# facebookresearch/omni3d

Measured on AMD Instinct MI355X. Metric: images/sec train DLA34_FPN b=4/GPU, higher is better.
Workload: dtype f32; 1 GPU; cubercnn_DLA34_FPN train step, batch 4/GPU, synthetic Omni3D 512x512 (8 GT/img), fwd+10 losses+bwd+allreduce+divergence guard+SGD, random-init weights; global_batch=4, image=512x512, parallelism=dp1 (flat-bucket RCCL all-reduce)

## Files before the change

include/omni3d_hip.h:

```cpp
#ifndef OMNI3D_HIP_H
#define OMNI3D_HIP_H

#ifdef __cplusplus
extern "C" {
#endif


int omni_iou_box3d(const float* boxes1, int N, const float* boxes2, int M, const int* valid1, float* vol,
                   float* iou, int* overflow, void* stream);

int omni_iou_box3d_pairs(const float* boxes1, const float* boxes2, const int* idx1, const int* idx2,
                         long long npairs, const int* valid1, float* vol, float* iou, int* overflow,
                         void* stream);

int omni_iou_box3d_pairs_algo(const float* boxes1, const float* boxes2, const int* idx1, const int* idx2,
                              long long npairs, const int* valid1, float* vol, float* iou, int* overflow,
                              int lanes_per_pair, void* stream);

int omni_box3d_validity(const float* boxes, int N, float eps_coplanar, float eps_nonzero, int* valid,
                        int* counts, void* stream);


int omni_conv2d_fwd(const float* x, const float* w, const float* bias, float* out, int N, int H, int W, int C,
                    int K, int R, int S, int stride, int pad, int ldx, int ldo, int relu, void* stream);
// ... 29 lines not shown
int omni_gemm_batched_split(const float* A, const float* B, float* out, int batch, int M, int N, int K, int terms, void* stream);
int omni_conv2d_s2_dgrad(const float* dy, const float* w, float* dx, int N, int H, int W, int C, int K, int lddy, int lddx,
                         int accumulate, void* stream);
int omni_conv2d_wgrad_multi_det(const void* const* xs, const int* cs, int nsrc, const float* dy, float* dw, int N, int H, int W, int K,
                                int lddy, int accumulate, int tile, float* ws, long long ws_floats, int* ctr, int n_ctr, long long* plan,
                                void* stream);


int omni_bn_fwd_algo(const float* x, const float* partial, int nblk, const float* gamma, const float* beta, const float* residual,
                     float* y, long long ldy, float* running_mean, float* running_var, float* mean_rstd, float* scale_shift,
                     double* ws, int P, int C, float eps, float momentum, int relu, int fuse_rows, void* stream);
int omni_bn_bwd_algo(const float* x, const float* dy, long long lddy, const float* y, const float* gamma, const float* mean_rstd,
                     const float* partial, int nblk, float* dx, float* dres, const float* res_carry, long long ldc, float* dgamma,
                     float* dbeta, double* ws, float* coef, int P, int C, int relu, int accumulate_param_grads, int fuse_rows,
                     void* stream);

int omni_bn_apply(const float* x, const float* scale_shift, const float* residual, float* y, int P, int C,
                  int relu, void* stream);

int omni_bn_frozen_fwd(const float* x, const float* gamma, const float* beta, const float* running_mean, const float* running_var,
                       float eps, const float* residual, float* y, int P, int C, int relu, void* stream);
int omni_bn_frozen_bwd(const float* x, const float* dy, long long lddy, const float* y, const float* gamma, const float* beta,
                       const float* running_mean, const float* running_var, float eps, float* dx, float* dres, const float* res_carry,
                       long long ldc, float* dgamma, float* dbeta, float* ws, long long ws_floats, int P, int C, int relu,
                       int accumulate_param_grads, void* stream);

int omni_maxpool2_fwd(const float* x, float* y, int N, int H, int W, int C, void* stream);
int omni_maxpool2_bwd(const float* x, const float* dy, float* dx, int N, int H, int W, int C, void* stream);

int omni_grouped_conv2d_fwd(const float* x, const float* w, float* out, int N, int H, int W, int C, int K, int R, int S, int stride,
// ... 272 lines not shown
```

omni3d_amd/csrc/bn_pool.hip:

```cpp
#include <device_rt.h>

namespace {

__device__ __forceinline__ float4 ld4(const float* p) { return *reinterpret_cast<const float4*>(p); }
__device__ __forceinline__ void st4(float* p, float4 v) { *reinterpret_cast<float4*>(p) = v; }
__device__ __forceinline__ float4 f4(float a) { return make_float4(a, a, a, a); }
__device__ __forceinline__ float4 relu4(float4 a) { return make_float4(fmaxf(a.x, 0.f), fmaxf(a.y, 0.f), fmaxf(a.z, 0.f), fmaxf(a.w, 0.f)); }
__device__ __forceinline__ float4 mask4(float4 g, float4 y) {
    return make_float4(y.x > 0.f ? g.x : 0.f, y.y > 0.f ? g.y : 0.f, y.z > 0.f ? g.z : 0.f, y.w > 0.f ? g.w : 0.f);
}

template <int MODE>
__device__ __forceinline__ void bn_reduce_tile(const float* __restrict__ x, const float* __restrict__ dy,
                                               const float* __restrict__ y, const float* __restrict__ mean_rstd,
                                               int P, int C, int relu, double* __restrict__ acc, int cbase, int C4,
                                               float4* __restrict__ s0, float4* __restrict__ s1, long lddy) {
    const int rows = 256 / C4;
    const int t = threadIdx.x;
    const int col = cbase + t % C4, row = t / C4;
    const bool active = row < rows;
    float4 a0 = f4(0.f), a1 = f4(0.f);
    float4 mu = f4(0.f), rs = f4(0.f), sc = f4(0.f), sh = f4(0.f);
    if (MODE == 1 && active) { mu = ld4(mean_rstd + 4 * col); rs = ld4(mean_rstd + C + 4 * col); }
    if (MODE == 1 && active && relu == 2) { sc = ld4(y + 4 * col); sh = ld4(y + C + 4 * col); }
// ... 343 lines not shown
        const float4 x0 = ld4(x + p * C + coff), x1 = two ? ld4(x + p1 * C + coff) : f4(0.f);
        if (relu == 1) {
            g0 = mask4(g0, ld4(y + p * C + coff));
            if (two) g1 = mask4(g1, ld4(y + p1 * C + coff));
        } else if (relu == 2) {
            g0 = mask4(g0, x0 * msc + msh);
            g1 = mask4(g1, x1 * msc + msh);
        }
        if (dres != nullptr) {
            st4(dres + p * C + coff, res_carry != nullptr ? g0 + ld4(res_carry + p * ldc + coff) : g0);
            if (two) st4(dres + p1 * C + coff, res_carry != nullptr ? g1 + ld4(res_carry + p1 * ldc + coff) : g1);
        }
        const float4 h0 = (x0 - mu) * rs, h1 = (x1 - mu) * rs;
        st4(dx + p * C + coff, k0 * (g0 - k1 - h0 * k2));
        if (two) st4(dx + p1 * C + coff, k0 * (g1 - k1 - h1 * k2));
    }
}

__device__ __forceinline__ float frozen_rsqrt(float v) {
#ifdef OMNI_HIPEMU
    return 1.f / sqrtf(v);
#else
    return rsqrtf(v);
#endif
}
__device__ __forceinline__ void frozen_coef(const float* __restrict__ gamma, const float* __restrict__ beta,
                                            const float* __restrict__ running_mean, const float* __restrict__ running_var, float eps,
                                            long c, float4& sc, float4& sh, float4& mu, float4& rs) {
#pragma clang fp contract(off)
    const float4 g = ld4(gamma + c), b = ld4(beta + c), v = ld4(running_var + c);
// ... 412 lines not shown
        int CG, PC, chunk, grid;
        fin_geometry(P, C, CG, PC, chunk, grid);
        hipLaunchKernelGGL(bn_fin_bwd_apply_kernel, dim3(grid), dim3(256), 0, st, x, dy, (long)lddy, y, mean_rstd, gamma, partial, nblk, P, C,
                           dgamma, dbeta, accumulate_param_grads, dx, dres, res_carry, (long)ldc, relu, CG, PC, chunk);
        return omni_launch_status();
    }
    if (coef == nullptr) return OMNI_ERR_ARG;
    hipLaunchKernelGGL(bn_finalize_bwd_kernel, dim3((C + FIN_C - 1) / FIN_C), dim3(256), 0, st, partial, nblk, P, C, gamma, mean_rstd,
                       dgamma, dbeta, coef, accumulate_param_grads);
    const long total4 = (long)P * (C >> 2);
    hipLaunchKernelGGL(bn_bwd_apply_kernel, dim3(ew_grid(total4)), dim3(256), 0, st, x, dy, y, mean_rstd,
                       (const float*)coef, dx, dres, total4, C, relu, res_carry, (long)ldc, (long)lddy);
    return omni_launch_status();
}

int omni_bn_frozen_fwd(const float* x, const float* gamma, const float* beta, const float* running_mean, const float* running_var,
                       float eps, const float* residual, float* y, int P, int C, int relu, void* stream) {
    if (P <= 0 || C <= 0 || (C & 3) || C > 4096 || !gamma || !beta || !running_mean || !running_var) return OMNI_ERR_ARG;
    int CG, PC, chunk, grid;
    fin_geometry(P, C, CG, PC, chunk, grid);
    hipLaunchKernelGGL(bn_frozen_fwd_kernel, dim3(grid), dim3(256), 0, (hipStream_t)stream, x, gamma, beta, running_mean, running_var, eps,
                       residual, y, P, C, relu, CG, PC, chunk);
    return omni_launch_status();
}

int omni_bn_frozen_bwd(const float* x, const float* dy, long long lddy, const float* y, const float* gamma, const float* beta,
                       const float* running_mean, const float* running_var, float eps, float* dx, float* dres, const float* res_carry,
                       long long ldc, float* dgamma, float* dbeta, float* ws, long long ws_floats, int P, int C, int relu,
                       int accumulate_param_grads, void* stream) {
    if (P <= 0 || C <= 0 || (C & 3) || C > 4096 || relu < 0 || relu > 2 || (relu == 1 && y == nullptr)) return OMNI_ERR_ARG;
// ... 163 lines not shown
```

omni3d_amd/csrc/winograd.hip:

```cpp
#include <device_rt.h>

namespace {

__device__ __forceinline__ float4 ld4(const float* p) { return *reinterpret_cast<const float4*>(p); }
__device__ __forceinline__ void st4(float* p, float4 v) { *reinterpret_cast<float4*>(p) = v; }
__device__ __forceinline__ float4 z4() { return make_float4(0.f, 0.f, 0.f, 0.f); }

inline int ew_grid(long total) {
    long g = (total + 255) / 256;
    if (g > 4096) g = 4096;
    return (int)(g < 1 ? 1 : g);
}

__device__ __forceinline__ float4 wino_ld(const float* __restrict__ p, bool ok, bool aff, float4 sc, float4 sh, int relu) {
    if (!ok) return z4();
    float4 v = ld4(p);
    if (aff) {
        v = v * sc + sh;
        if (relu) v = make_float4(fmaxf(v.x, 0.f), fmaxf(v.y, 0.f), fmaxf(v.z, 0.f), fmaxf(v.w, 0.f));
    }
    return v;
}

__global__ void __launch_bounds__(256) wino_in_kernel(const float* __restrict__ x, float* __restrict__ V, int N, int H, int W,
// ... 226 lines not shown
__global__ void __launch_bounds__(256) wino_dw_kernel(const float* __restrict__ dU, float* __restrict__ dg, int K, int C,
                                                      int accumulate) {
#pragma clang fp contract(off)
    const long total = (long)K * C;
    for (long i = (long)blockIdx.x * blockDim.x + threadIdx.x; i < total; i += (long)gridDim.x * blockDim.x) {
        const int c = (int)(i % C), k = (int)(i / C);
        float v[3][3];
        wino_dw_elem(dU, total, i, v);
#pragma unroll
        for (int r = 0; r < 3; ++r) {
            float* o = dg + ((long)k * 9 + r * 3) * C + c;
            if (accumulate) { o[0] += v[r][0]; o[C] += v[r][1]; o[2 * (long)C] += v[r][2]; }
            else { o[0] = v[r][0]; o[C] = v[r][1]; o[2 * (long)C] = v[r][2]; }
        }
    }
}

template <typename V>
__device__ __forceinline__ void bt6(const V (&d)[6], V (&t)[6]) {
    t[0] = d[0] + (d[3] - d[1]) * 1.5f - d[2] * 2.f + d[4];
    t[1] = d[2] * 0.5f + d[3] * 2.5f - d[1] + d[4];
    t[2] = d[1] - d[2] * 2.5f + d[3] * 0.5f + d[4];
    t[3] = (d[3] - d[1]) * 2.f - d[2] + d[4];
    t[4] = (d[1] - d[3]) * 0.5f - d[2] + d[4];
    t[5] = d[1] + (d[4] - d[2]) * 1.5f - d[3] * 2.f + d[5];
}
template <typename V>
__device__ __forceinline__ void at6(const V (&m)[6], V (&y)[4]) {
    y[0] = m[0] + m[1] + m[2] + m[3] + m[4];
    y[1] = m[1] - m[2] + m[3] * 0.5f - m[4] * 2.f;
    y[2] = m[1] + m[2] + m[3] * 0.25f + m[4] * 4.f;
    y[3] = m[1] - m[2] + m[3] * 0.125f - m[4] * 8.f + m[5];
}
template <typename V>
__device__ __forceinline__ void a6(const V (&y)[4], V (&u)[6]) {
    u[0] = y[0];
    u[1] = y[0] + y[1] + y[2] + y[3];
    u[2] = y[0] - y[1] + y[2] - y[3];
    u[3] = y[0] + y[1] * 0.5f + y[2] * 0.25f + y[3] * 0.125f;
    u[4] = y[0] - y[1] * 2.f + y[2] * 4.f - y[3] * 8.f;
    u[5] = y[3];
}

__global__ void __launch_bounds__(256) wino4_in_kernel(const float* __restrict__ x, float* __restrict__ V, int N, int H, int W,
                                                       int C, const float* __restrict__ affine, int relu, long plane_in) {
    const int C4 = C >> 2, TH = H >> 2, TW = W >> 2;
    const bool aff = affine != nullptr;
    const long T = (long)N * TH * TW, total = T * C4, plane = plane_in > 0 ? plane_in : T * C;
    for (long i = (long)blockIdx.x * blockDim.x + threadIdx.x; i < total; i += (long)gridDim.x * blockDim.x) {
        const int c4 = (int)(i % C4);
        const long t = i / C4;
        const int tx = (int)(t % TW);
        const int ty = (int)((t / TW) % TH);
        const int n = (int)(t / ((long)TW * TH));
        const float4 sc = aff ? ld4(affine + 4 * c4) : z4(), sh = aff ? ld4(affine + C + 4 * c4) : z4();
        float4 u[6][6];
// ... 337 lines not shown
        const long t = i / K4;
        const int tx = (int)(t % TW);
        const int ty = (int)((t / TW) % TH);
        const int n = (int)(t / ((long)TW * TH));
        float4 d[4][4];
#pragma unroll
        for (int r = 0; r < 4; ++r) {
            const int ih = 2 * ty - 1 + r;
#pragma unroll
            for (int s = 0; s < 4; ++s) {
                const int iw = 2 * tx - 1 + s;
                const bool ok = (unsigned)ih < (unsigned)H && (unsigned)iw < (unsigned)W;
                d[r][s] = ok ? ld4(dy + (((long)n * H + ih) * W + iw) * K + 4 * k4) : z4();
            }
        }
        const long o = t * K + 4 * k4;
        {
            float4 u[4][4];
#pragma unroll
            for (int s = 0; s < 4; ++s) {
                u[0][s] = d[0][s] - d[2][s];
                u[1][s] = d[1][s] + d[2][s];
                u[2][s] = d[2][s] - d[1][s];
                u[3][s] = d[1][s] - d[3][s];
            }
#pragma unroll
            for (int r = 0; r < 4; ++r) {
                st4(Vd + o + (long)(4 * r + 0) * plane, u[r][0] - u[r][2]);
                st4(Vd + o + (long)(4 * r + 1) * plane, u[r][1] + u[r][2]);
                st4(Vd + o + (long)(4 * r + 2) * plane, u[r][2] - u[r][1]);
                st4(Vd + o + (long)(4 * r + 3) * plane, u[r][1] - u[r][3]);
            }
        }
        {
            const float4 g00 = d[1][1], g01 = d[1][2], g10 = d[2][1], g11 = d[2][2];
            float4 u[4][2];
            u[0][0] = g00;        u[0][1] = g01;
            u[1][0] = g00 + g10;  u[1][1] = g01 + g11;
            u[2][0] = g00 - g10;  u[2][1] = g01 - g11;
            u[3][0] = z4() - g10; u[3][1] = z4() - g11;
#pragma unroll
            for (int r = 0; r < 4; ++r) {
                st4(dM + o + (long)(4 * r + 0) * plane, u[r][0]);
                st4(dM + o + (long)(4 * r + 1) * plane, u[r][0] + u[r][1]);
                st4(dM + o + (long)(4 * r + 2) * plane, u[r][0] - u[r][1]);
                st4(dM + o + (long)(4 * r + 3) * plane, z4() - u[r][1]);
            }
        }
    }
}

__global__ void __launch_bounds__(256) wino4_dy_in_kernel(const float* __restrict__ dy, float* __restrict__ dM, float* __restrict__ Vd,
                                                          int N, int H, int W, int K, long plane_in) {
    const int K4 = K >> 2, TH = H >> 2, TW = W >> 2;
    const long T = (long)N * TH * TW, total = T * K4, plane = plane_in > 0 ? plane_in : T * K;
    for (long i = (long)blockIdx.x * blockDim.x + threadIdx.x; i < total; i += (long)gridDim.x * blockDim.x) {
        const int k4 = (int)(i % K4);
        const long t = i / K4;
        const int tx = (int)(t % TW);
        const int ty = (int)((t / TW) % TH);
        const int n = (int)(t / ((long)TW * TH));
        float4 d[6][6];
#pragma unroll
        for (int r = 0; r < 6; ++r) {
            const int ih = 4 * ty - 1 + r;
#pragma unroll
            for (int s = 0; s < 6; ++s) {
                const int iw = 4 * tx - 1 + s;
                const bool ok = (unsigned)ih < (unsigned)H && (unsigned)iw < (unsigned)W;
                d[r][s] = ok ? ld4(dy + (((long)n * H + ih) * W + iw) * K + 4 * k4) : z4();
            }
        }
        const long o = t * K + 4 * k4;
        {
            float4 u[6][4];
#pragma unroll
            for (int c = 0; c < 4; ++c) {
                float4 col[4], o6[6];
#pragma unroll
                for (int r = 0; r < 4; ++r) col[r] = d[1 + r][1 + c];
                a6(col, o6);
#pragma unroll
                for (int r = 0; r < 6; ++r) u[r][c] = o6[r];
            }
#pragma unroll
            for (int r = 0; r < 6; ++r) {
                float4 row[6];
                a6(u[r], row);
#pragma unroll
                for (int c = 0; c < 6; ++c) st4(dM + o + (long)(6 * r + c) * plane, row[c]);
            }
        }
        {
            float4 u[6][6];
#pragma unroll
            for (int s = 0; s < 6; ++s) {
                float4 col[6], tcol[6];
#pragma unroll
                for (int r = 0; r < 6; ++r) col[r] = d[r][s];
                bt6(col, tcol);
#pragma unroll
                for (int r = 0; r < 6; ++r) u[r][s] = tcol[r];
            }
#pragma unroll
            for (int r = 0; r < 6; ++r) {
                float4 v[6];
                bt6(u[r], v);
#pragma unroll
                for (int s = 0; s < 6; ++s) st4(Vd + o + (long)(6 * r + s) * plane, v[s]);
            }
        }
    }
}

inline bool bad(int N, int H, int W, int C) { return N < 0 || H <= 0 || W <= 0 || C <= 0 || (C & 3); }

}

extern "C" {

int omni_wino_in(const float* x, float* V, int N, int H, int W, int C, int tile, void* stream) {
    if (bad(N, H, W, C) || (tile != 2 && tile != 4) || (H % tile) || (W % tile)) return OMNI_ERR_ARG;
    const long total = (long)N * (H / tile) * (W / tile) * (C / 4);
    if (total == 0) return OMNI_OK;
    const float* affine = nullptr;
    const long plane = 0;
// ... 133 lines not shown
```

omni3d_amd/functional.py:

```python
import torch
from torch.autograd import Function
from os import environ as _environ

_os_environ_get = _environ.get

from .kernels import glue
from .kernels import bnpool, conv, det, wino

CL = torch.channels_last


def _cl(t):
    return t if t.is_contiguous(memory_format=CL) else t.contiguous(memory_format=CL)


def _direct_grad(t):
    if t is not None and getattr(t, "_omni_direct_grad", False) and t.grad is not None and t.requires_grad:
        return t.grad
    return None


def _parts_out(parts, like):
    return parts if parts is not None else like.new_zeros((0, 1))

# ... 255 lines not shown
        cache = _wino_scope["cache"]
        U, Uf = cache.get(key, (None, None)) if cache is not None else (None, None)
        if U is None or (need_flip and Uf is None):
            U, Uf = wino.transform_weights(w, True, need_flip or Uf is not None, tile)
            if cache is not None:
                cache[key] = (U, Uf)
                if w is w_given:
                    _wino_scope["record"].append((w, tile, bool(need_flip or Uf is not None)))
        parts = None
        if want_stats and bias is None and not relu:
            y, V, parts = wino.conv3x3_fwd(x, w, None, False, U=U, tile=tile, want_stats=True)
        else:
            y, V = wino.conv3x3_fwd(x, w, bias, relu, U=U, tile=tile)
        ctx.save_for_backward(V, w, y if relu else None, Uf if need_flip else None)
        ctx.cfg = (relu, bias is not None)
        parts = _parts_out(parts, y)
        ctx.mark_non_differentiable(parts)
        return y, parts

    @staticmethod
    def backward(ctx, dy, _parts_grad=None):
        V, w, y, Uf = ctx.saved_tensors
        relu, has_bias = ctx.cfg
        relu = relu and not _relu_already_masked(dy)
        dy = _cl(dy)
        if relu:
            dy = bnpool.relu_bwd(dy.permute(0, 2, 3, 1), y.permute(0, 2, 3, 1)).permute(0, 3, 1, 2)
        gw, gb = ctx.direct
        if gw is not None and not gw.is_contiguous(memory_format=CL):
            gw = None
        dx = dw = None
        slot, box = ctx.slot, []

        def fused(carry):
            ok = carry is not None and _carry_pitch(carry) is not None
            dx_, dw_ = wino.conv3x3_backward(V, dy, w, Uf, accum_into=gw, side_run=_side_run, bn_below=ctx.bn_below if carry is None else None,
                                             carry=carry if ok else None)
            box.append(dw_)
            return dx_ if (ok or carry is None) else dx_ + carry

        def dgrad_only(carry):
            if wino.dgrad_eligible(dy.shape):
                ok = carry is not None and _carry_pitch(carry) is not None
                dx_ = wino.conv3x3_dgrad(dy, w, U_flip=Uf, tile=2 if V.shape[0] == 16 else 4, carry=carry if ok else None)
                return dx_ if (ok or carry is None) else dx_ + carry
            if carry is not None and _carry_pitch(carry) is not None:
                return conv.conv2d_dgrad(dy, w, (dy.shape[2], dy.shape[3]), 1, 1, accum_into=carry)
            return _add_carry(conv.conv2d_dgrad(dy, w, (dy.shape[2], dy.shape[3]), 1, 1), carry)

        if ctx.needs_input_grad[0] and ctx.needs_input_grad[1] and wino.dgrad_eligible(dy.shape):
            dx = _slot_deliver(slot, fused)
            dw = box[0]
# ... 80 lines not shown
            for w, tile, flip in record:
                old = plan.get((id(w), tile))
                plan[(id(w), tile)] = (w, tile, flip or (old[2] if old else False))
            try:
                object.__setattr__(self.owner, self.kind, list(plan.values()))
            except Exception:
                pass
        _wino_scope["cache"], _wino_scope["record"] = self.prev
        return False



def conv2d(x, w, bias=None, stride=1, pad=0, relu=False, want_stats=False):
    if wino.eligible(x.shape, w.shape, stride, pad):
        y, parts = _WinoConv3x3.apply(x, w, bias, relu, want_stats)
    else:
        y, parts = _Conv2d.apply(x, w, bias, stride, pad, relu, want_stats)
    if parts.shape[0] > 0:
        y._omni_bn_partials = parts
    return y


class _GroupedConv2d(Function):
    @staticmethod
    def forward(ctx, x, w, groups, stride, pad):
        x, w = _cl(x), _cl(w)
        ctx.save_for_backward(x, w)
        ctx.cfg = (groups, stride, pad)
        return conv.grouped_conv2d_fwd(x, w, groups, stride, pad)

# ... 77 lines not shown
    pad = rows - sum(w.shape[0] for w in weights)
    w = torch.cat(list(weights) + ([weights[0].new_zeros(pad, cols)] if pad else []), dim=0)
    b = torch.cat(list(biases) + ([biases[0].new_zeros(pad)] if pad else []), dim=0)
    return _Linear.apply(x, w, b, relu, None, None)


_BN_BWD_FUSE = _os_environ_get("OMNI_BN_BWD_FUSE", "1") != "0"


class _BatchNorm(Function):
    @staticmethod
    def forward(ctx, x, gamma, beta, running_mean, running_var, residual, relu, eps, momentum, partials=None):
        gg, gb = _direct_grad(gamma), _direct_grad(beta)
        ctx.direct = (gg, gb) if (gg is not None and gb is not None) else None
        ctx.res_slot = _slot_enter(residual, residual is not None and ctx.needs_input_grad[5])
        x = _cl(x)
        res = _cl(residual) if residual is not None else None
        y, mean_rstd, scale_shift = bnpool.bn_fwd(x, gamma, beta, running_mean, running_var, res, relu, eps, momentum, partials)
        remask = relu and residual is None
        ctx.save_for_backward(x, gamma, mean_rstd, (y if relu and not remask else None), (scale_shift if remask else None))
        ctx.cfg = (relu, residual is not None)
        if _BN_BWD_FUSE and residual is None and (remask or not relu):
            y._omni_bn_below = (x, mean_rstd, scale_shift if relu else None)
        return y

    @staticmethod
    def backward(ctx, dy):
        x, gamma, mean_rstd, y, scale_shift = ctx.saved_tensors
        relu, has_res = ctx.cfg
        parts = getattr(dy, "_omni_bn_bwd_parts", None)
        if parts is not None:
            parts = parts[0] if parts[1].data_ptr() == mean_rstd.data_ptr() and dy.is_contiguous(memory_format=CL) else None
        want_dres = has_res and ctx.needs_input_grad[5]
        box = []

        dyk = dy if (parts is None and not dy.is_contiguous(memory_format=CL) and _carry_pitch(dy) is not None) else _cl(dy)

        def run(carry):
            ok = carry is not None and parts is None and _carry_pitch(carry) is not None
            dx_, dres_, dgamma_, dbeta_ = bnpool.bn_bwd(x, dyk, y, gamma, mean_rstd, relu, want_dres=want_dres, accum_into=ctx.direct,
                                                        scale_shift=scale_shift, partials=parts, res_carry=carry if ok else None)
            box.append((dx_, dgamma_, dbeta_))
            return dres_ if (ok or carry is None) else dres_ + carry

        dres = _slot_deliver(ctx.res_slot, run) if want_dres else run(None)
        dx, dgamma, dbeta = box[0]
        return dx, dgamma, dbeta, None, None, dres, None, None, None, None


def batch_norm_train(x, gamma, beta, running_mean, running_var, residual=None, relu=False, eps=1e-5, momentum=0.1):
    return _BatchNorm.apply(x, gamma, beta, running_mean, running_var, residual, relu, eps, momentum, getattr(x, "_omni_bn_partials", None))


class _FrozenBatchNorm(Function):

    @staticmethod
    def forward(ctx, x, gamma, beta, running_mean, running_var, residual, relu, eps):
        gg, gb = _direct_grad(gamma), _direct_grad(beta)
        ctx.direct = (gg, gb) if (gg is not None and gb is not None) else None
        ctx.res_slot = _slot_enter(residual, residual is not None and ctx.needs_input_grad[5])
        x = _cl(x)
# ... 521 lines not shown
```

omni3d_amd/kernels/bnpool.py:

```python
import torch

from .. import lib as _lib
from .conv import _nhwc


def _like_cl(shape_nhwc, ref):
    return torch.empty(shape_nhwc, dtype=torch.float32, device=ref.device)


FUSE_ROWS = 512


def _pitched_out(out, N, H, W, C):
    assert tuple(out.shape) == (N, C, H, W) and out.dtype == torch.float32 and out.stride(1) == 1, (out.shape, out.stride())
    ldy = out.stride(3)
    assert out.stride(2) == W * ldy and out.stride(0) == H * W * ldy and ldy >= C and ldy % 4 == 0 and out.data_ptr() % 16 == 0
    return out, out.data_ptr(), ldy


def bn_fwd(x, gamma, beta, running_mean, running_var, residual=None, relu=False, eps=1e-5, momentum=0.1, partials=None, out=None):
    xv = _nhwc(x)
    rv = _nhwc(residual) if residual is not None else None
    N, H, W, C = xv.shape
    L = _lib.check_device(xv, rv, gamma, beta, running_mean, running_var)
# ... 63 lines not shown
            dgamma, dbeta = accum_into
            assert dgamma.is_contiguous() and dbeta.is_contiguous() and dgamma.numel() == C and dbeta.numel() == C
        else:
            dgamma = torch.empty(C, dtype=torch.float32, device=x.device)
            dbeta = torch.empty(C, dtype=torch.float32, device=x.device)
        ws = torch.empty(2 * C * 512, dtype=torch.float32, device=x.device)
    L.call("omni_bn_frozen_bwd", _lib.ptr(xv), dy.data_ptr() if dy_pitched else _lib.ptr(dyv), dy.stride(3) if dy_pitched else C, _lib.ptr(yv),
           _lib.ptr(gamma), _lib.ptr(beta), _lib.ptr(running_mean), _lib.ptr(running_var), float(eps), _lib.ptr(dx), _lib.ptr(dres),
           _lib.ptr(res_carry), res_carry.stride(3) if res_carry is not None else 0, _lib.ptr(dgamma), _lib.ptr(dbeta), _lib.ptr(ws),
           ws.numel() if ws is not None else 0, N * H * W, C, mode, int(accum_into is not None), _lib.stream_of(x))
    if accum_into is not None:
        dgamma = dbeta = None
    return dx.permute(0, 3, 1, 2), (dres.permute(0, 3, 1, 2) if want_dres else None), dgamma, dbeta


def bn_bwd(x, dy, y, gamma, mean_rstd, relu=False, want_dres=False, accum_into=None, scale_shift=None, partials=None, res_carry=None):
    xv = _nhwc(x)
    dy_pitched = not dy.is_contiguous(memory_format=torch.channels_last)
    dyv = None if dy_pitched else _nhwc(dy)
    mode = int(bool(relu))
    if relu and scale_shift is not None:
        assert y is None and scale_shift.is_contiguous() and scale_shift.numel() == 2 * xv.shape[3]
        yv, mode = scale_shift, 2
    else:
        yv = _nhwc(y) if relu else None
    N, H, W, C = xv.shape
    L = _lib.check_device(xv, dyv, yv, gamma, mean_rstd)
    dx = _like_cl((N, H, W, C), x)
    dres = _like_cl((N, H, W, C), x) if want_dres else None
    if accum_into is not None:
        dgamma, dbeta = accum_into
        assert dgamma.is_contiguous() and dbeta.is_contiguous()
    else:
        dgamma = torch.empty(C, dtype=torch.float32, device=x.device)
        dbeta = torch.empty(C, dtype=torch.float32, device=x.device)
    coef = torch.empty(3 * C, dtype=torch.float32, device=x.device)
    ws = None
    if partials is not None:
        assert partials.is_contiguous() and partials.shape[1] == 2 * C and res_carry is None and not dy_pitched
    else:
        ws = torch.empty(2 * C * 258, dtype=torch.float64, device=x.device)
    if res_carry is not None or dy_pitched:
        assert tuple(dy.shape) == tuple(x.shape) and dy.stride(1) == 1
        if res_carry is not None:
            assert want_dres and tuple(res_carry.shape) == tuple(x.shape)
    L.call("omni_bn_bwd_algo", _lib.ptr(xv), dy.data_ptr() if dy_pitched else _lib.ptr(dyv), dy.stride(3) if dy_pitched else C, _lib.ptr(yv),
           _lib.ptr(gamma), _lib.ptr(mean_rstd), _lib.ptr(partials), partials.shape[0] if partials is not None else 0, _lib.ptr(dx),
           _lib.ptr(dres), _lib.ptr(res_carry), res_carry.stride(3) if res_carry is not None else 0, _lib.ptr(dgamma), _lib.ptr(dbeta),
           _lib.ptr(ws), _lib.ptr(coef), N * H * W, C, mode, int(accum_into is not None), FUSE_ROWS, _lib.stream_of(x))
    if accum_into is not None:
        dgamma = dbeta = None
    return dx.permute(0, 3, 1, 2), (dres.permute(0, 3, 1, 2) if want_dres else None), dgamma, dbeta


def _simple(name, src, out_shape, dims, extra_in=()):
    L = _lib.check_device(src, *extra_in)
    out = torch.empty(out_shape, dtype=torch.float32, device=src.device)
    L.call(name, *[_lib.ptr(t) for t in (src, *extra_in)], _lib.ptr(out), *dims, _lib.stream_of(src))
    return out


def maxpool2_fwd(x):
    xv = _nhwc(x)
    N, H, W, C = xv.shape
    return _simple("omni_maxpool2_fwd", xv, (N, H // 2, W // 2, C), (N, H, W, C)).permute(0, 3, 1, 2)


# ... 140 lines not shown
```

omni3d_amd/kernels/wino.py:

```python
import torch

from .. import lib as _lib
from . import detmode as _det

CL = torch.channels_last


import os as _os

_F43_MIN_TILES = 256
_MIN_TILES = 256
_DGRAD_MIN_TILES = 256


def eligible(x_shape, w_shape, stride, pad):
    N, C, H, W = x_shape
    K, _, R, S = w_shape
    if not (R == 3 and S == 3 and stride == 1 and pad == 1 and H % 2 == 0 and W % 2 == 0 and C % 32 == 0 and K % 32 == 0):
        return False
    if C >= 128 and K >= 128 and N * (H // 2) * (W // 2) >= _MIN_TILES:
        return True
    return C >= 64 and K >= 64 and tile_size(x_shape) == 4 and N * (H // 4) * (W // 4) >= 4096


# ... 273 lines not shown
    Mt = gemm_batched(V, U)
    if want_stats:
        y, parts = transform_output_stats(Mt, (N, H, W))
        return y, V, parts
    return transform_output(Mt, (N, H, W), bias, relu), V


def conv3x3_dgrad(dy, w, U_flip=None, tile=2, carry=None):
    N, _, H, W = dy.shape
    if U_flip is None:
        U_flip = transform_weights(w, want_u=False, want_flip=True, tile=tile)[1]
    Mt = gemm_batched(transform_input(dy, tile), U_flip)
    return transform_output(Mt, (N, H, W), carry=carry)


def conv3x3_backward(V, dy, w, U_flip, accum_into=None, side_run=None, bn_below=None, carry=None):
    N, _, H, W = dy.shape
    tile = 2 if V.shape[0] == 16 else 4
    dM, Vd = transform_dy_both(dy, tile)
    if side_run is not None and accum_into is not None:
        dw = side_run(lambda: wgrad_into(V, dM, accum_into), (V, dM))
    else:
        dw = None
    if U_flip is None:
        U_flip = transform_weights(w, want_u=False, want_flip=True, tile=tile)[1]
    if carry is not None:
        dx = transform_output(gemm_batched(Vd, U_flip), (N, H, W), carry=carry)
    elif bn_below is not None and tile == 4:
        dx, parts = transform_output_bn_bwd(gemm_batched(Vd, U_flip), (N, H, W), *bn_below[:3])
        if parts is not None:
            dx._omni_bn_bwd_parts = (parts, bn_below[1])
    else:
        dx = transform_output(gemm_batched(Vd, U_flip), (N, H, W))
    if side_run is None or accum_into is None:
# ... 10 lines not shown
```

Measured before the change: 380.1 images/s.

## Fuse BatchNorm backward finalize with Winograd dy transform of the conv above

When a BatchNorm directly follows a Winograd 3x3 conv (no bias/relu), the BN backward kernel now writes the Winograd-transformed dM and Vd planes for that conv's backward, instead of materializing dx in NHWC. The conv backward then takes these planes and skips its own transform_dy_both pass. This removes one full write and read of the gradient tensor plus a kernel launch. In exchange the BN kernel re-reads overlapping tile halos, and a runtime guard is needed because the conv output must have no second consumer.

Measured after the change: 367.6 images/s. 3.3% lower.

```diff
diff --git a/include/omni3d_hip.h b/include/omni3d_hip.h
--- a/include/omni3d_hip.h
+++ b/include/omni3d_hip.h
@@ -67,6 +67,10 @@
                      const float* partial, int nblk, float* dx, float* dres, const float* res_carry, long long ldc, float* dgamma,
                      float* dbeta, double* ws, float* coef, int P, int C, int relu, int accumulate_param_grads, int fuse_rows,
                      void* stream);
+int omni_bn_bwd_wino_dy(const float* x, const float* dy, long long lddy, const float* y, const float* gamma, const float* mean_rstd,
+                        const float* partial, int nblk, float* dres, const float* res_carry, long long ldc, float* dgamma,
+                        float* dbeta, double* ws, float* dM, float* Vd, int N, int H, int W, int C, int tile, int relu,
+                        int accumulate_param_grads, void* stream);
 
 int omni_bn_apply(const float* x, const float* scale_shift, const float* residual, float* y, int P, int C,
                   int relu, void* stream);
diff --git a/omni3d_amd/csrc/bn_pool.hip b/omni3d_amd/csrc/bn_pool.hip
--- a/omni3d_amd/csrc/bn_pool.hip
+++ b/omni3d_amd/csrc/bn_pool.hip
@@ -1,4 +1,5 @@
 #include <device_rt.h>
+#include "wino_tf.h"
 
 namespace {
 
@@ -381,6 +382,77 @@
         const float4 h0 = (x0 - mu) * rs, h1 = (x1 - mu) * rs;
         st4(dx + p * C + coff, k0 * (g0 - k1 - h0 * k2));
         if (two) st4(dx + p1 * C + coff, k0 * (g1 - k1 - h1 * k2));
+    }
+}
+
+#ifdef OMNI_HIPEMU
+#define OMNI_OPAQUE4(v) do { } while (0)
+#else
+#define OMNI_OPAQUE4(v) asm volatile("" : "+v"((v).x), "+v"((v).y), "+v"((v).z), "+v"((v).w))
+#endif
+template <int TILE>
+__global__ void __launch_bounds__(256) bn_fin_bwd_wino_dy_kernel(const float* __restrict__ x, const float* __restrict__ dy, long lddy,
+                                                                 const float* __restrict__ y, const float* __restrict__ mean_rstd,
+                                                                 const float* __restrict__ gamma, const float* __restrict__ partial,
+                                                                 int nblk, int P, int C, float* __restrict__ dgamma,
+                                                                 float* __restrict__ dbeta, int accumulate, float* __restrict__ dres,
+                                                                 const float* __restrict__ res_carry, long ldc, int relu,
+                                                                 float* __restrict__ dM, float* __restrict__ Vd, int N, int H, int W,
+                                                                 int CG, int PC, int chunk) {
+    constexpr int F = TILE + 2;
+    int cg, pc;
+    if (!fin_item(CG, PC, cg, pc)) return;
+    const int c0 = cg * GC, t = threadIdx.x;
+    __shared__ float s_cf[3 * GC];
+    double db, dg;
+    colsum_fin_quads(partial, nblk, C, c0, db, dg);
+    if (t < GC) {
+        const int c = c0 + t;
+        if (pc == 0) {
+            dbeta[c] = accumulate ? dbeta[c] + (float)db : (float)db;
+            dgamma[c] = accumulate ? dgamma[c] + (float)dg : (float)dg;
+        }
+        s_cf[t] = gamma[c] * mean_rstd[C + c];
+        s_cf[GC + t] = (float)(db / P);
+        s_cf[2 * GC + t] = (float)(dg / P);
+    }
+    __syncthreads();
+    const int col = t & (GQ - 1), trow = t >> 2;
+    const long coff = c0 + 4 * col;
+    const float4 k0 = ld4(s_cf + 4 * col), k1 = ld4(s_cf + GC + 4 * col), k2 = ld4(s_cf + 2 * GC + 4 * col);
+    const float4 mu = ld4(mean_rstd + coff), rs = ld4(mean_rstd + C + coff);
+    float4 msc = f4(0.f), msh = f4(0.f);
+    if (relu == 2) { msc = ld4(y + coff); msh = ld4(y + C + coff); }
+    const int TH = H / TILE, TW = W / TILE;
+    const long T = (long)N * TH * TW, plane = T * C;
+    const long tend = min(T, (long)(pc + 1) * chunk);
+    for (long tl = (long)pc * chunk + trow; tl < tend; tl += 64) {
+        const int tx = (int)(tl % TW);
+        const int ty = (int)((tl / TW) % TH);
+        const int n = (int)(tl / ((long)TW * TH));
+        float4 d[F][F];
+#pragma unroll
+        for (int r = 0; r < F; ++r) {
+            const int ih = TILE * ty - 1 + r;
+#pragma unroll
+            for (int s = 0; s < F; ++s) {
+                const int iw = TILE * tx - 1 + s;
+                const bool ok = (unsigned)ih < (unsigned)H && (unsigned)iw < (unsigned)W;
+                const long p = ((long)n * H + ih) * W + iw;
+                float4 g = ok ? ld4(dy + p * lddy + coff) : f4(0.f);
+                const float4 xv = ok ? ld4(x + p * C + coff) : f4(0.f);
+                if (relu == 1) g = mask4(g, ok ? ld4(y + p * C + coff) : f4(0.f));
+                else if (relu == 2) g = mask4(g, xv * msc + msh);
+                if (r >= 1 && r <= TILE && s >= 1 && s <= TILE && dres != nullptr)
+                    st4(dres + p * C + coff, res_carry != nullptr ? g + ld4(res_carry + p * ldc + coff) : g);
+                const float4 h = (xv - mu) * rs;
+                float4 v = k0 * (g - k1 - h * k2);
+                OMNI_OPAQUE4(v);
+                d[r][s] = ok ? v : f4(0.f);
+            }
+        }
+        if constexpr (TILE == 2) wino2_dy_both_store(d, dM, Vd, tl * C + coff, plane);
+        else wino4_dy_both_store(d, dM, Vd, tl * C + coff, plane);
     }
 }
 
@@ -823,6 +895,38 @@
     return omni_launch_status();
 }
 
+int omni_bn_bwd_wino_dy(const float* x, const float* dy, long long lddy, const float* y, const float* gamma, const float* mean_rstd,
+                        const float* partial, int nblk, float* dres, const float* res_carry, long long ldc, float* dgamma, float* dbeta,
+                        double* ws, float* dM, float* Vd, int N, int H, int W, int C, int tile, int relu, int accumulate_param_grads,
+                        void* stream) {
+    if (N <= 0 || H <= 0 || W <= 0 || C <= 0 || (C % GC) || C > 4096 || relu < 0 || relu > 2 || (relu && y == nullptr)) return OMNI_ERR_ARG;
+    if ((tile != 2 && tile != 4) || (H % tile) || (W % tile) || dM == nullptr || Vd == nullptr) return OMNI_ERR_ARG;
+    const long P = (long)N * H * W, T = (long)N * (H / tile) * (W / tile);
+    if (P > 0x7fffffffL) return OMNI_ERR_ARG;
+    if (lddy == 0) lddy = C;
+    if (bad_carry(res_carry, ldc, C) || (res_carry != nullptr && dres == nullptr) || bad_carry(dy, lddy, C)) return OMNI_ERR_ARG;
+    if ((partial != nullptr && (nblk <= 0 || res_carry != nullptr || lddy != C)) || (partial == nullptr && ws == nullptr)) return OMNI_ERR_ARG;
+    hipStream_t st = (hipStream_t)stream;
+    if (partial == nullptr) {
+        nblk = red_grid((int)P, C);
+        float* mine = reinterpret_cast<float*>(ws + 2 * C);
+        hipLaunchKernelGGL(HIP_KERNEL_NAME(bn_reduce_kernel<1>), dim3(nblk), dim3(256), 0, st, x, dy, y, mean_rstd, (int)P, C, relu,
+                           reinterpret_cast<double*>(mine), (long)lddy);
+        partial = mine;
+    }
+    int CG, PC, chunk, grid;
+    fin_geometry((int)T, C, CG, PC, chunk, grid);
+    if (tile == 2)
+        hipLaunchKernelGGL(HIP_KERNEL_NAME(bn_fin_bwd_wino_dy_kernel<2>), dim3(grid), dim3(256), 0, st, x, dy, (long)lddy, y, mean_rstd, gamma,
+                           partial, nblk, (int)P, C, dgamma, dbeta, accumulate_param_grads, dres, res_carry, (long)ldc, relu, dM, Vd, N, H, W,
+                           CG, PC, chunk);
+    else
+        hipLaunchKernelGGL(HIP_KERNEL_NAME(bn_fin_bwd_wino_dy_kernel<4>), dim3(grid), dim3(256), 0, st, x, dy, (long)lddy, y, mean_rstd, gamma,
+                           partial, nblk, (int)P, C, dgamma, dbeta, accumulate_param_grads, dres, res_carry, (long)ldc, relu, dM, Vd, N, H, W,
+                           CG, PC, chunk);
+    return omni_launch_status();
+}
+
 int omni_bn_frozen_fwd(const float* x, const float* gamma, const float* beta, const float* running_mean, const float* running_var,
                        float eps, const float* residual, float* y, int P, int C, int relu, void* stream) {
     if (P <= 0 || C <= 0 || (C & 3) || C > 4096 || !gamma || !beta || !running_mean || !running_var) return OMNI_ERR_ARG;
diff --git a/omni3d_amd/csrc/wino_tf.h b/omni3d_amd/csrc/wino_tf.h
--- /dev/null
+++ b/omni3d_amd/csrc/wino_tf.h
@@ -0,0 +1,109 @@
+#pragma once
+#include <device_rt.h>
+
+template <typename V>
+__device__ __forceinline__ void bt6(const V (&d)[6], V (&t)[6]) {
+    t[0] = d[0] + (d[3] - d[1]) * 1.5f - d[2] * 2.f + d[4];
+    t[1] = d[2] * 0.5f + d[3] * 2.5f - d[1] + d[4];
+    t[2] = d[1] - d[2] * 2.5f + d[3] * 0.5f + d[4];
+    t[3] = (d[3] - d[1]) * 2.f - d[2] + d[4];
+    t[4] = (d[1] - d[3]) * 0.5f - d[2] + d[4];
+    t[5] = d[1] + (d[4] - d[2]) * 1.5f - d[3] * 2.f + d[5];
+}
+template <typename V>
+__device__ __forceinline__ void at6(const V (&m)[6], V (&y)[4]) {
+    y[0] = m[0] + m[1] + m[2] + m[3] + m[4];
+    y[1] = m[1] - m[2] + m[3] * 0.5f - m[4] * 2.f;
+    y[2] = m[1] + m[2] + m[3] * 0.25f + m[4] * 4.f;
+    y[3] = m[1] - m[2] + m[3] * 0.125f - m[4] * 8.f + m[5];
+}
+template <typename V>
+__device__ __forceinline__ void a6(const V (&y)[4], V (&u)[6]) {
+    u[0] = y[0];
+    u[1] = y[0] + y[1] + y[2] + y[3];
+    u[2] = y[0] - y[1] + y[2] - y[3];
+    u[3] = y[0] + y[1] * 0.5f + y[2] * 0.25f + y[3] * 0.125f;
+    u[4] = y[0] - y[1] * 2.f + y[2] * 4.f - y[3] * 8.f;
+    u[5] = y[3];
+}
+
+__device__ __forceinline__ void wino_tf_st4(float* p, float4 v) { *reinterpret_cast<float4*>(p) = v; }
+__device__ __forceinline__ float4 wino_tf_z4() { return make_float4(0.f, 0.f, 0.f, 0.f); }
+
+__device__ __forceinline__ void wino2_dy_both_store(const float4 (&d)[4][4], float* __restrict__ dM, float* __restrict__ Vd, long o,
+                                                    long plane) {
+    {
+        float4 u[4][4];
+#pragma unroll
+        for (int s = 0; s < 4; ++s) {
+            u[0][s] = d[0][s] - d[2][s];
+            u[1][s] = d[1][s] + d[2][s];
+            u[2][s] = d[2][s] - d[1][s];
+            u[3][s] = d[1][s] - d[3][s];
+        }
+#pragma unroll
+        for (int r = 0; r < 4; ++r) {
+            wino_tf_st4(Vd + o + (long)(4 * r + 0) * plane, u[r][0] - u[r][2]);
+            wino_tf_st4(Vd + o + (long)(4 * r + 1) * plane, u[r][1] + u[r][2]);
+            wino_tf_st4(Vd + o + (long)(4 * r + 2) * plane, u[r][2] - u[r][1]);
+            wino_tf_st4(Vd + o + (long)(4 * r + 3) * plane, u[r][1] - u[r][3]);
+        }
+    }
+    {
+        const float4 g00 = d[1][1], g01 = d[1][2], g10 = d[2][1], g11 = d[2][2];
+        float4 u[4][2];
+        u[0][0] = g00;                  u[0][1] = g01;
+        u[1][0] = g00 + g10;            u[1][1] = g01 + g11;
+        u[2][0] = g00 - g10;            u[2][1] = g01 - g11;
+        u[3][0] = wino_tf_z4() - g10;   u[3][1] = wino_tf_z4() - g11;
+#pragma unroll
+        for (int r = 0; r < 4; ++r) {
+            wino_tf_st4(dM + o + (long)(4 * r + 0) * plane, u[r][0]);
+            wino_tf_st4(dM + o + (long)(4 * r + 1) * plane, u[r][0] + u[r][1]);
+            wino_tf_st4(dM + o + (long)(4 * r + 2) * plane, u[r][0] - u[r][1]);
+            wino_tf_st4(dM + o + (long)(4 * r + 3) * plane, wino_tf_z4() - u[r][1]);
+        }
+    }
+}
+
+__device__ __forceinline__ void wino4_dy_both_store(const float4 (&d)[6][6], float* __restrict__ dM, float* __restrict__ Vd, long o,
+                                                    long plane) {
+    {
+        float4 u[6][4];
+#pragma unroll
+        for (int c = 0; c < 4; ++c) {
+            float4 col[4], o6[6];
+#pragma unroll
+            for (int r = 0; r < 4; ++r) col[r] = d[1 + r][1 + c];
+            a6(col, o6);
+#pragma unroll
+            for (int r = 0; r < 6; ++r) u[r][c] = o6[r];
+        }
+#pragma unroll
+        for (int r = 0; r < 6; ++r) {
+            float4 row[6];
+            a6(u[r], row);
+#pragma unroll
+            for (int c = 0; c < 6; ++c) wino_tf_st4(dM + o + (long)(6 * r + c) * plane, row[c]);
+        }
+    }
+    {
+        float4 u[6][6];
+#pragma unroll
+        for (int s = 0; s < 6; ++s) {
+            float4 col[6], tcol[6];
+#pragma unroll
+            for (int r = 0; r < 6; ++r) col[r] = d[r][s];
+            bt6(col, tcol);
+#pragma unroll
+            for (int r = 0; r < 6; ++r) u[r][s] = tcol[r];
+        }
+#pragma unroll
+        for (int r = 0; r < 6; ++r) {
+            float4 v[6];
+            bt6(u[r], v);
+#pragma unroll
+            for (int s = 0; s < 6; ++s) wino_tf_st4(Vd + o + (long)(6 * r + s) * plane, v[s]);
+        }
+    }
+}
diff --git a/omni3d_amd/csrc/winograd.hip b/omni3d_amd/csrc/winograd.hip
--- a/omni3d_amd/csrc/winograd.hip
+++ b/omni3d_amd/csrc/winograd.hip
@@ -1,4 +1,5 @@
 #include <device_rt.h>
+#include "wino_tf.h"
 
 namespace {
 
@@ -264,32 +265,6 @@
             else { o[0] = v[r][0]; o[C] = v[r][1]; o[2 * (long)C] = v[r][2]; }
         }
     }
-}
-
-template <typename V>
-__device__ __forceinline__ void bt6(const V (&d)[6], V (&t)[6]) {
-    t[0] = d[0] + (d[3] - d[1]) * 1.5f - d[2] * 2.f + d[4];
-    t[1] = d[2] * 0.5f + d[3] * 2.5f - d[1] + d[4];
-    t[2] = d[1] - d[2] * 2.5f + d[3] * 0.5f + d[4];
-    t[3] = (d[3] - d[1]) * 2.f - d[2] + d[4];
-    t[4] = (d[1] - d[3]) * 0.5f - d[2] + d[4];
-    t[5] = d[1] + (d[4] - d[2]) * 1.5f - d[3] * 2.f + d[5];
-}
-template <typename V>
-__device__ __forceinline__ void at6(const V (&m)[6], V (&y)[4]) {
-    y[0] = m[0] + m[1] + m[2] + m[3] + m[4];
-    y[1] = m[1] - m[2] + m[3] * 0.5f - m[4] * 2.f;
-    y[2] = m[1] + m[2] + m[3] * 0.25f + m[4] * 4.f;
-    y[3] = m[1] - m[2] + m[3] * 0.125f - m[4] * 8.f + m[5];
-}
-template <typename V>
-__device__ __forceinline__ void a6(const V (&y)[4], V (&u)[6]) {
-    u[0] = y[0];
-    u[1] = y[0] + y[1] + y[2] + y[3];
-    u[2] = y[0] - y[1] + y[2] - y[3];
-    u[3] = y[0] + y[1] * 0.5f + y[2] * 0.25f + y[3] * 0.125f;
-    u[4] = y[0] - y[1] * 2.f + y[2] * 4.f - y[3] * 8.f;
-    u[5] = y[3];
 }
 
 __global__ void __launch_bounds__(256) wino4_in_kernel(const float* __restrict__ x, float* __restrict__ V, int N, int H, int W,
@@ -657,39 +632,7 @@
                 d[r][s] = ok ? ld4(dy + (((long)n * H + ih) * W + iw) * K + 4 * k4) : z4();
             }
         }
-        const long o = t * K + 4 * k4;
-        {
-            float4 u[4][4];
-#pragma unroll
-            for (int s = 0; s < 4; ++s) {
-                u[0][s] = d[0][s] - d[2][s];
-                u[1][s] = d[1][s] + d[2][s];
-                u[2][s] = d[2][s] - d[1][s];
-                u[3][s] = d[1][s] - d[3][s];
-            }
-#pragma unroll
-            for (int r = 0; r < 4; ++r) {
-                st4(Vd + o + (long)(4 * r + 0) * plane, u[r][0] - u[r][2]);
-                st4(Vd + o + (long)(4 * r + 1) * plane, u[r][1] + u[r][2]);
-                st4(Vd + o + (long)(4 * r + 2) * plane, u[r][2] - u[r][1]);
-                st4(Vd + o + (long)(4 * r + 3) * plane, u[r][1] - u[r][3]);
-            }
-        }
-        {
-            const float4 g00 = d[1][1], g01 = d[1][2], g10 = d[2][1], g11 = d[2][2];
-            float4 u[4][2];
-            u[0][0] = g00;        u[0][1] = g01;
-            u[1][0] = g00 + g10;  u[1][1] = g01 + g11;
-            u[2][0] = g00 - g10;  u[2][1] = g01 - g11;
-            u[3][0] = z4() - g10; u[3][1] = z4() - g11;
-#pragma unroll
-            for (int r = 0; r < 4; ++r) {
-                st4(dM + o + (long)(4 * r + 0) * plane, u[r][0]);
-                st4(dM + o + (long)(4 * r + 1) * plane, u[r][0] + u[r][1]);
-                st4(dM + o + (long)(4 * r + 2) * plane, u[r][0] - u[r][1]);
-                st4(dM + o + (long)(4 * r + 3) * plane, z4() - u[r][1]);
-            }
-        }
+        wino2_dy_both_store(d, dM, Vd, t * K + 4 * k4, plane);
     }
 }
 
@@ -714,45 +657,7 @@
                 d[r][s] = ok ? ld4(dy + (((long)n * H + ih) * W + iw) * K + 4 * k4) : z4();
             }
         }
-        const long o = t * K + 4 * k4;
-        {
-            float4 u[6][4];
-#pragma unroll
-            for (int c = 0; c < 4; ++c) {
-                float4 col[4], o6[6];
-#pragma unroll
-                for (int r = 0; r < 4; ++r) col[r] = d[1 + r][1 + c];
-                a6(col, o6);
-#pragma unroll
-                for (int r = 0; r < 6; ++r) u[r][c] = o6[r];
-            }
-#pragma unroll
-            for (int r = 0; r < 6; ++r) {
-                float4 row[6];
-                a6(u[r], row);
-#pragma unroll
-                for (int c = 0; c < 6; ++c) st4(dM + o + (long)(6 * r + c) * plane, row[c]);
-            }
-        }
-        {
-            float4 u[6][6];
-#pragma unroll
-            for (int s = 0; s < 6; ++s) {
-                float4 col[6], tcol[6];
-#pragma unroll
-                for (int r = 0; r < 6; ++r) col[r] = d[r][s];
-                bt6(col, tcol);
-#pragma unroll
-                for (int r = 0; r < 6; ++r) u[r][s] = tcol[r];
-            }
-#pragma unroll
-            for (int r = 0; r < 6; ++r) {
-                float4 v[6];
-                bt6(u[r], v);
-#pragma unroll
-                for (int s = 0; s < 6; ++s) st4(Vd + o + (long)(6 * r + s) * plane, v[s]);
-            }
-        }
+        wino4_dy_both_store(d, dM, Vd, t * K + 4 * k4, plane);
     }
 }
 
diff --git a/omni3d_amd/functional.py b/omni3d_amd/functional.py
--- a/omni3d_amd/functional.py
+++ b/omni3d_amd/functional.py
@@ -293,6 +293,9 @@
             y, V = wino.conv3x3_fwd(x, w, bias, relu, U=U, tile=tile)
         ctx.save_for_backward(V, w, y if relu else None, Uf if need_flip else None)
         ctx.cfg = (relu, bias is not None)
+        ctx.planes_tile = tile if (bias is None and not relu and ctx.needs_input_grad[0] and ctx.needs_input_grad[1]
+                                   and wino.dgrad_eligible(y.shape)) else None
+        ctx.planes_sent = False
         parts = _parts_out(parts, y)
         ctx.mark_non_differentiable(parts)
         return y, parts
@@ -301,8 +304,14 @@
     def backward(ctx, dy, _parts_grad=None):
         V, w, y, Uf = ctx.saved_tensors
         relu, has_bias = ctx.cfg
+        planes = getattr(dy, "_omni_dy_planes", None)
+        if ctx.planes_sent and planes is None:
+            raise RuntimeError("omni3d_amd: the output of a convolution whose BatchNorm hands its gradient over in transformed form "
+                               "(functional._BatchNorm.backward) has a second consumer")
+        ctx.planes_sent = False
         relu = relu and not _relu_already_masked(dy)
-        dy = _cl(dy)
+        if planes is None:
+            dy = _cl(dy)
         if relu:
             dy = bnpool.relu_bwd(dy.permute(0, 2, 3, 1), y.permute(0, 2, 3, 1)).permute(0, 3, 1, 2)
         gw, gb = ctx.direct
@@ -314,7 +323,7 @@
         def fused(carry):
             ok = carry is not None and _carry_pitch(carry) is not None
             dx_, dw_ = wino.conv3x3_backward(V, dy, w, Uf, accum_into=gw, side_run=_side_run, bn_below=ctx.bn_below if carry is None else None,
-                                             carry=carry if ok else None)
+                                             carry=carry if ok else None, planes=planes)
             box.append(dw_)
             return dx_ if (ok or carry is None) else dx_ + carry
 
@@ -425,6 +434,8 @@
 def conv2d(x, w, bias=None, stride=1, pad=0, relu=False, want_stats=False):
     if wino.eligible(x.shape, w.shape, stride, pad):
         y, parts = _WinoConv3x3.apply(x, w, bias, relu, want_stats)
+        if want_stats and y.grad_fn is not None and getattr(y.grad_fn, "planes_tile", None) is not None:
+            y._omni_wino_above = y.grad_fn
     else:
         y, parts = _Conv2d.apply(x, w, bias, stride, pad, relu, want_stats)
     if parts.shape[0] > 0:
@@ -532,6 +543,7 @@
         gg, gb = _direct_grad(gamma), _direct_grad(beta)
         ctx.direct = (gg, gb) if (gg is not None and gb is not None) else None
         ctx.res_slot = _slot_enter(residual, residual is not None and ctx.needs_input_grad[5])
+        ctx.wino_above = getattr(x, "_omni_wino_above", None) if bnpool.wino_dy_fusable(x.shape[1]) else None
         x = _cl(x)
         res = _cl(residual) if residual is not None else None
         y, mean_rstd, scale_shift = bnpool.bn_fwd(x, gamma, beta, running_mean, running_var, res, relu, eps, momentum, partials)
@@ -557,12 +569,19 @@
         def run(carry):
             ok = carry is not None and parts is None and _carry_pitch(carry) is not None
             dx_, dres_, dgamma_, dbeta_ = bnpool.bn_bwd(x, dyk, y, gamma, mean_rstd, relu, want_dres=want_dres, accum_into=ctx.direct,
-                                                        scale_shift=scale_shift, partials=parts, res_carry=carry if ok else None)
+                                                        scale_shift=scale_shift, partials=parts, res_carry=carry if ok else None,
+                                                        wino_tile=above.planes_tile if above is not None else None)
             box.append((dx_, dgamma_, dbeta_))
             return dres_ if (ok or carry is None) else dres_ + carry
 
+        above = ctx.wino_above
         dres = _slot_deliver(ctx.res_slot, run) if want_dres else run(None)
         dx, dgamma, dbeta = box[0]
+        if above is not None:
+            planes = dx
+            dx = planes[0].new_empty(1).as_strided(x.shape, (0, 0, 0, 0))
+            dx._omni_dy_planes = planes
+            above.planes_sent = True
         return dx, dgamma, dbeta, None, None, dres, None, None, None, None
 
 
diff --git a/omni3d_amd/kernels/bnpool.py b/omni3d_amd/kernels/bnpool.py
--- a/omni3d_amd/kernels/bnpool.py
+++ b/omni3d_amd/kernels/bnpool.py
@@ -101,7 +101,12 @@
     return dx.permute(0, 3, 1, 2), (dres.permute(0, 3, 1, 2) if want_dres else None), dgamma, dbeta
 
 
-def bn_bwd(x, dy, y, gamma, mean_rstd, relu=False, want_dres=False, accum_into=None, scale_shift=None, partials=None, res_carry=None):
+def wino_dy_fusable(C):
+    return C % 16 == 0
+
+
+def bn_bwd(x, dy, y, gamma, mean_rstd, relu=False, want_dres=False, accum_into=None, scale_shift=None, partials=None, res_carry=None,
+           wino_tile=None):
     xv = _nhwc(x)
     dy_pitched = not dy.is_contiguous(memory_format=torch.channels_last)
     dyv = None if dy_pitched else _nhwc(dy)
@@ -113,7 +118,6 @@
         yv = _nhwc(y) if relu else None
     N, H, W, C = xv.shape
     L = _lib.check_device(xv, dyv, yv, gamma, mean_rstd)
-    dx = _like_cl((N, H, W, C), x)
     dres = _like_cl((N, H, W, C), x) if want_dres else None
     if accum_into is not None:
         dgamma, dbeta = accum_into
@@ -121,7 +125,6 @@
     else:
         dgamma = torch.empty(C, dtype=torch.float32, device=x.device)
         dbeta = torch.empty(C, dtype=torch.float32, device=x.device)
-    coef = torch.empty(3 * C, dtype=torch.float32, device=x.device)
     ws = None
     if partials is not None:
         assert partials.is_contiguous() and partials.shape[1] == 2 * C and res_carry is None and not dy_pitched
@@ -131,13 +134,27 @@
         assert tuple(dy.shape) == tuple(x.shape) and dy.stride(1) == 1
         if res_carry is not None:
             assert want_dres and tuple(res_carry.shape) == tuple(x.shape)
+    if accum_into is not None:
+        ret_dgamma = ret_dbeta = None
+    else:
+        ret_dgamma, ret_dbeta = dgamma, dbeta
+    if wino_tile is not None:
+        assert wino_dy_fusable(C) and H % wino_tile == 0 and W % wino_tile == 0
+        shape = ((wino_tile + 2) ** 2, N * (H // wino_tile) * (W // wino_tile), C)
+        dM = torch.empty(shape, dtype=torch.float32, device=x.device)
+        Vd = torch.empty(shape, dtype=torch.float32, device=x.device)
+        L.call("omni_bn_bwd_wino_dy", _lib.ptr(xv), dy.data_ptr() if dy_pitched else _lib.ptr(dyv), dy.stride(3) if dy_pitched else C,
+               _lib.ptr(yv), _lib.ptr(gamma), _lib.ptr(mean_rstd), _lib.ptr(partials), partials.shape[0] if partials is not None else 0,
+               _lib.ptr(dres), _lib.ptr(res_carry), res_carry.stride(3) if res_carry is not None else 0, _lib.ptr(dgamma), _lib.ptr(dbeta),
+               _lib.ptr(ws), _lib.ptr(dM), _lib.ptr(Vd), N, H, W, C, wino_tile, mode, int(accum_into is not None), _lib.stream_of(x))
+        return (dM, Vd), (dres.permute(0, 3, 1, 2) if want_dres else None), ret_dgamma, ret_dbeta
+    dx = _like_cl((N, H, W, C), x)
+    coef = torch.empty(3 * C, dtype=torch.float32, device=x.device)
     L.call("omni_bn_bwd_algo", _lib.ptr(xv), dy.data_ptr() if dy_pitched else _lib.ptr(dyv), dy.stride(3) if dy_pitched else C, _lib.ptr(yv),
            _lib.ptr(gamma), _lib.ptr(mean_rstd), _lib.ptr(partials), partials.shape[0] if partials is not None else 0, _lib.ptr(dx),
            _lib.ptr(dres), _lib.ptr(res_carry), res_carry.stride(3) if res_carry is not None else 0, _lib.ptr(dgamma), _lib.ptr(dbeta),
            _lib.ptr(ws), _lib.ptr(coef), N * H * W, C, mode, int(accum_into is not None), FUSE_ROWS, _lib.stream_of(x))
-    if accum_into is not None:
-        dgamma = dbeta = None
-    return dx.permute(0, 3, 1, 2), (dres.permute(0, 3, 1, 2) if want_dres else None), dgamma, dbeta
+    return dx.permute(0, 3, 1, 2), (dres.permute(0, 3, 1, 2) if want_dres else None), ret_dgamma, ret_dbeta
 
 
 def _simple(name, src, out_shape, dims, extra_in=()):
diff --git a/omni3d_amd/kernels/wino.py b/omni3d_amd/kernels/wino.py
--- a/omni3d_amd/kernels/wino.py
+++ b/omni3d_amd/kernels/wino.py
@@ -311,10 +311,10 @@
     return transform_output(Mt, (N, H, W), carry=carry)
 
 
-def conv3x3_backward(V, dy, w, U_flip, accum_into=None, side_run=None, bn_below=None, carry=None):
+def conv3x3_backward(V, dy, w, U_flip, accum_into=None, side_run=None, bn_below=None, carry=None, planes=None):
     N, _, H, W = dy.shape
     tile = 2 if V.shape[0] == 16 else 4
-    dM, Vd = transform_dy_both(dy, tile)
+    dM, Vd = planes if planes is not None else transform_dy_both(dy, tile)
     if side_run is not None and accum_into is not None:
         dw = side_run(lambda: wgrad_into(V, dM, accum_into), (V, dM))
     else:
```
